# mgp25/OpenLTE

Measured on AMD Instinct MI355X. Metric: DL subframes/sec @20MHz 100RB 64QAM, full chain FFT->CE->demap->rate-unmatch->turbo(REF)->CRC (SURVEY 8d W4), higher is better.
Workload: dtype i8 IQ in, f32 FFT/CE/equaliser, i8 soft bits, i16 path metrics (differences exact modulo 2^16); 1 GPU; W4 full DL chain: 20 MHz/100 RB/64QAM, 9 allocations per subframe (8x12 PRB TBS 3240 + 1x4 PRB TBS 1064), 65536 subframes per GPU, int8 IQ in HBM; subframes_per_gpu=65536, N_ant=1, CFI=2, channel_estimate_form=compact, decoder=REF (reference-faithful, bit-exact), unique_subframes=96, streams_per_gpu=1

## Files before the change

openlte_amd/csrc/turbo.hip:

```cpp
#include <algorithm>
#include <cstring>
#include <initializer_list>
#include <type_traits>
#include <vector>

#include "plan_core.hpp"
#include "turbo_swar.h"
#include "soft_pack.h"

using namespace turbo_geom;

namespace {

constexpr uint32_t RX_NULL_AS_INT = 10000;


__device__ __forceinline__ int sbyte(uint32_t w, int k) { return (int)__builtin_amdgcn_sbfe(w, 8 * k, 8); }

typedef __attribute__((address_space(3))) const uint8_t  lds_u8_t;
typedef __attribute__((address_space(3))) const int8_t   lds_i8_t;
typedef __attribute__((address_space(3))) const uint16_t lds_u16_t;
__device__ __forceinline__ uint32_t lds_u8(uint32_t addr) { return *(lds_u8_t *)(uintptr_t)addr; }
__device__ __forceinline__ int      lds_i8(uint32_t addr) { return *(lds_i8_t *)(uintptr_t)addr; }
__device__ __forceinline__ uint32_t lds_u16(uint32_t addr) { return *(lds_u16_t *)(uintptr_t)addr; }
// ... 641 lines not shown
    __syncthreads();

    uint4 I0 = make_uint4(0, 0, 0, 0);
    if (nv > 0) {
        uint32_t idx[16];
        if constexpr (MULTI)
            load_idx16_at(reinterpret_cast<const_u32x4_t *>(reinterpret_cast<uintptr_t>(pi + 16 * (size_t)u)), nv, idx, K);
        else
            load_idx16(pi, u, nv, idx, K);
        I0 = gather16_bytes(PREP_Q0_AT, idx);
    }
    if (nv >= 0) *reinterpret_cast<uint4 *>(out.arr[3] + unit_off(tile_off, lane, u)) = I0;
    if (identity && src.hard_inputs()) {
        auto cnt4 = [](uint32_t a, uint32_t b) { return (a & 0x01010101u) + (b & 0x01010101u); };
        const uint32_t c1[4] = {cnt4(Q[1].x, Q[0].x), cnt4(Q[1].y, Q[0].y), cnt4(Q[1].z, Q[0].z), cnt4(Q[1].w, Q[0].w)};
        const uint32_t c2[4] = {cnt4(Q[2].x, I0.x), cnt4(Q[2].y, I0.y), cnt4(Q[2].z, I0.z), cnt4(Q[2].w, I0.w)};
        const uint32_t o1 = c1[0] | c1[1] | c1[2] | c1[3], o2 = c2[0] | c2[1] | c2[2] | c2[3];
        int w1max = (o1 & 0x02020202u) ? 254 : (o1 ? 127 : 0), w2max = (o2 & 0x02020202u) ? 254 : (o2 ? 127 : 0);
        block_max_i2(w1max, w2max, red_i);
        if (w1max != 0 && w2max != 0) {
            auto mag4 = [](uint32_t cnt, int W) { return W == 254 ? (cnt << 6) - ((cnt | (cnt >> 1)) & 0x01010101u) : (cnt << 7) - cnt; };
            if (nv >= 0) {
                *reinterpret_cast<uint4 *>(out.arr[4] + unit_off(tile_off, lane, u)) = make_uint4(mag4(c1[0], w1max), mag4(c1[1], w1max), mag4(c1[2], w1max), mag4(c1[3], w1max));
                *reinterpret_cast<uint4 *>(out.arr[5] + unit_off(tile_off, lane, u)) = make_uint4(mag4(c2[0], w2max), mag4(c2[1], w2max), mag4(c2[2], w2max), mag4(c2[3], w2max));
            }
            return;
        }
    }
    uint32_t w1[16], w2[16], w1m = 0, w2m = 0;
    abs_sum16(Q[1], Q[0], w1, w1m);
    abs_sum16(Q[2], I0, w2, w2m);
    int w1max = (int)w1m, w2max = (int)w2m;
    block_max_i2(w1max, w2max, red_i);
    auto closed = [](int W) { return W == 254 || W == 127; };
    auto closed16 = [](const uint32_t (&w)[16], int W) {
        uint32_t o[4];
#pragma unroll
        for (int j = 0; j < 4; j++) {
            const uint32_t p = pack4u(w[4 * j], w[4 * j + 1], w[4 * j + 2], w[4 * j + 3]);
            o[j] = W == 254 ? (p >> 1) & 0x7F7F7F7Fu : p;
        }
        return make_uint4(o[0], o[1], o[2], o[3]);
    };
    if (!(closed(w1max) && closed(w2max))) {
        const float W1 = (float)w1max, W2 = (float)w2max;
        for (uint32_t t = threadIdx.x; t < MTAB_N; t += blockDim.x) {
            const float w = (float)t;
            mtab1[t] = (int8_t)(int)(127.0f * (w / W1));
            mtab2[t] = (int8_t)(int)(127.0f * (w / W2));
        }
        __syncthreads();
    }
    if (nv >= 0) {
        *reinterpret_cast<uint4 *>(out.arr[4] + unit_off(tile_off, lane, u)) = closed(w1max) ? closed16(w1, w1max) : lookup16(0, w1);
        *reinterpret_cast<uint4 *>(out.arr[5] + unit_off(tile_off, lane, u)) = closed(w2max) ? closed16(w2, w2max) : lookup16(MTAB_N, w2);
    }
}


struct SisoPass {
    const uint8_t *in_a;
    const uint8_t *in_b;
    uint32_t      *sgn;
    uint32_t      *dec;
};
struct SisoArgs { SisoPass p[2]; };

typedef unsigned short v2u __attribute__((ext_vector_type(2)));
__device__ __forceinline__ uint32_t sign_bits(v2s n) { return __builtin_bit_cast(uint32_t, __builtin_bit_cast(v2u, n) >> 15); }

template <int S> __device__ __forceinline__ void acs_step2(v2s (&pm)[8], v2s x2, v2s y2, uint32_t &acc)
{
    const v2s mx = as_v2s(neg_mask(x2 ^ y2)), nmx = ~mx;
    const v2s uP = (x2 + y2) & nmx;
    const v2s uQ = (x2 - y2) & mx;
    const uint32_t m0p = neg_mask(x2) & 0xFFF8FFF8u;
    const v2s P2 = as_v2s(__builtin_amdgcn_bitop3_b32(as_u32(mx), m0p, 0xFFFCFFFCu, 0x06));
    const v2s Q2 = as_v2s(__builtin_amdgcn_bitop3_b32(as_u32(mx), m0p, 0xFFFCFFFCu, 0x60));
    const v2s n0 = pm[1] - pm[0], n1 = pm[3] - pm[2], n2 = pm[5] - pm[4], n3 = pm[7] - pm[6];
    constexpr uint32_t top = 0x00010001u << (15 - 4 * S);
    acc = __builtin_amdgcn_bitop3_b32(acc, neg_mask(n0), top, 0xF8);
    acc = __builtin_amdgcn_bitop3_b32(acc, neg_mask(n1), top >> 1, 0xF8);
// ... 338 lines not shown
            G = map_compose(G, map_row_shl<2>(G, MAP_ID));
            G = map_compose(G, map_row_shl<4>(G, MAP_ID));
            G = map_compose(G, map_row_shl<8>(G, MAP_ID));
            const uint32_t row = lane >> 4;
#pragma unroll
            for (int r = 1; r < 4; r++) {
                const uint2 R = make_uint2((uint32_t)__builtin_amdgcn_readlane((int)G.x, 16 * r), (uint32_t)__builtin_amdgcn_readlane((int)G.y, 16 * r));
                if (row < (uint32_t)r) G = map_compose(G, R);
            }
            const uint2    Gn  = make_uint2((uint32_t)__shfl_down((int)G.x, 1u), (uint32_t)__shfl_down((int)G.y, 1u));
            const uint32_t nxt = lane == 63 ? end : map_at(Gn, end);
            const uint32_t st  = map_at(G, end);
            const bool     pos = (nxt < st) || (nxt == st && nxt == 0);
            const uint64_t neg = __ballot(__shfl((int)(t < K && !pos), (int)turbo_swar::sign_plane_lane(lane)) != 0);
            if (lane == 0) *reinterpret_cast<uint2 *>(sgn + 2 * ch) = make_uint2((uint32_t)neg, (uint32_t)(neg >> 32));
            end = (uint32_t)__builtin_amdgcn_readlane((int)st, 0);
        }
    }
}

namespace sw = turbo_swar;
struct UnitWords { uint32_t w[5]; };
__device__ __forceinline__ UnitWords load_unit_words(const uint8_t *arr, size_t tile_off, uint32_t lane, uint32_t u)
{
    const uint4 c    = *reinterpret_cast<const uint4 *>(arr + unit_off(tile_off, lane, u));
    uint32_t    prev = 0x7F7F7F7Fu;
    if (u > 0) prev = *reinterpret_cast<const uint32_t *>(arr + unit_off(tile_off, lane, u - 1) + 12);
    return UnitWords{{prev, c.x, c.y, c.z, c.w}};
}
struct UnitSigned {
    uint32_t halo, m[4], x;
    __device__ __forceinline__ sw::SM4 word(int j) const { return sw::SM4{m[j], sw::signed_under(m[j], x, j)}; }
};
__device__ __forceinline__ UnitSigned load_unit_signed(const uint8_t *mag, const uint32_t *sgn, size_t tile_off, uint32_t lane, uint32_t nblk, uint32_t u)
{
    const UnitWords w  = load_unit_words(mag, tile_off, lane, u);
    const uint32_t *sp = sgn + (tile_off >> 5) + sw::sign_word_index(lane, nblk, u >> 1);
    const uint32_t  S = sp[0];
    uint32_t        Sb = 0;
    if ((u & 1u) == 0 && u > 0) Sb = sp[-1];
    UnitSigned r{w.w[0], {w.w[1], w.w[2], w.w[3], w.w[4]}, sw::sign_unit(S, u)};
    if (u > 0) r.halo |= sw::signed_under_flags(r.halo, sw::sign_halo(S, Sb, u));
    return r;
}
struct PermArgs { const uint8_t *M1; const uint32_t *S1;  const uint8_t *X2; uint8_t *out[2];  };

#ifndef PERM_NB
#define PERM_NB 4
#endif
static_assert(PERM_NB == PERM_BLOCKS, "a size's perm grid is a multiple of 128 workgroups (the merged decode's map granularity) only for four blocks per workgroup");
template <int NSLOT, bool MULTI = false>
__global__ __launch_bounds__(384) void k_turbo_perm(PermArgs a, uint32_t K_arg, uint32_t n_cb_arg, const uint16_t *__restrict__ pi_arg, MultiArgs ma)
{
    static_assert(NSLOT == 1, "one unit per thread");
    uint32_t K = K_arg, n_cb = n_cb_arg, bidx = blockIdx.x, grid = gridDim.x;
    size_t   seg_off = 0;
    const uint16_t *__restrict__ pi = pi_arg;
    if constexpr (MULTI) {
        const_seg_t &sg = multi_seg(ma, blockIdx.x >> 7);
        K = sg.K; n_cb = sg.n_cb; pi = (const uint16_t *)sg.pi; bidx = blockIdx.x - sg.wg_perm; grid = sg.perm_grid;
        seg_off = sg.arr_off;
    }
    extern __shared__ __attribute__((aligned(16))) int8_t smp[];
    int8_t *mtab = smp, *sm = smp + MTAB_N;
    const uint32_t Kp = kpad64(K), n_units = Kp >> 4;
    int           *red_i = reinterpret_cast<int *>(sm + Kp);
    const uint32_t u0 = threadIdx.x;
    const int      nv = (u0 < n_units) ? min(16, max(0, (int)K - 16 * (int)u0)) : -1;
    IdxRaw         praw;
    {
        const uint4 *ip = reinterpret_cast<const uint4 *>(pi + 16 * (size_t)(nv > 0 ? u0 : 0));
        const uint32_t kk = K | K << 16;
        praw.lo = ip[0];
        praw.hi = (nv > 8) ? ip[1] : make_uint4(kk, kk, kk, kk);
    }
#pragma unroll 1
    for (uint32_t it = 0; it < PERM_NB; it++) {
        const uint32_t cb = xcd_cb(bidx + it * grid, n_cb), tile = cb >> 6, lane = cb & 63;
        const size_t   tile_off = seg_off + (size_t)tile * Kp * 64;
        if (cb >= n_cb) {
            if (MULTI && cb < ((n_cb + 63u) & ~63u) && nv >= 0) {
                *reinterpret_cast<uint4 *>(a.out[0] + unit_off(tile_off, lane, u0)) = make_uint4(0, 0, 0, 0);
                *reinterpret_cast<uint4 *>(a.out[1] + unit_off(tile_off, lane, u0)) = make_uint4(0, 0, 0, 0);
            }
            continue;
        }
        uint32_t u = u0;
        asm volatile("" : "+v"(u), "+v"(praw.lo.x), "+v"(praw.lo.y), "+v"(praw.lo.z), "+v"(praw.lo.w), "+v"(praw.hi.x), "+v"(praw.hi.y), "+v"(praw.hi.z), "+v"(praw.hi.w));
        uint4          X2 = make_uint4(0, 0, 0, 0);
        if (nv >= 0) {
            const UnitSigned ua = load_unit_signed(a.M1, a.S1, tile_off, lane, n_units >> 2, u);
            uint32_t         pa = ua.halo;
            X2 = *reinterpret_cast<const uint4 *>(a.X2 + unit_off(tile_off, lane, u));
            uint32_t c1[4];
#pragma unroll
            for (int j = 0; j < 4; j++) {
                const sw::SM4  A  = ua.word(j);
                const uint32_t ja = sw::join(A);
                c1[j] = (4 * j < nv) ? sw::to_tc(sw::step3(A, sw::feedback(ja, pa))) : 0u;
                pa    = ja;
            }
            *reinterpret_cast<uint4 *>(sm + 16 * u) = make_uint4(c1[0], c1[1], c1[2], c1[3]);
        }
        __syncthreads();
        uint4 I1 = make_uint4(0, 0, 0, 0);
        if (nv > 0) {
            uint32_t idx[16];
            unpack_idx16(praw, idx);
            I1 = gather16_bytes(MTAB_N, idx);
        }
        if (nv >= 0) *reinterpret_cast<uint4 *>(a.out[0] + unit_off(tile_off, lane, u)) = I1;
        uint32_t w[16], wm = 0;
        if (nv <= 0) X2 = make_uint4(0, 0, 0, 0);
        abs_sum16(X2, I1, w, wm);
        const int   wmax = block_max_i((int)wm, red_i);
        if (wmax == 254 || wmax == 127) {
            uint32_t o[4];
#pragma unroll
            for (int j = 0; j < 4; j++) {
                const uint32_t p = pack4u(w[4 * j], w[4 * j + 1], w[4 * j + 2], w[4 * j + 3]);
                o[j] = wmax == 254 ? (p >> 1) & 0x7F7F7F7Fu : p;
            }
            if (nv >= 0) *reinterpret_cast<uint4 *>(a.out[1] + unit_off(tile_off, lane, u)) = make_uint4(o[0], o[1], o[2], o[3]);
            continue;
        }
        const float W = (float)wmax;
        for (uint32_t t = threadIdx.x; t < MTAB_N; t += blockDim.x) mtab[t] = (int8_t)(int)(127.0f * ((float)t / W));
        __syncthreads();
        if (nv >= 0) *reinterpret_cast<uint4 *>(a.out[1] + unit_off(tile_off, lane, u)) = lookup16(0, w);
        __syncthreads();
    }
}

struct VoteArgs { const uint8_t *X0, *M1, *M2, *M3; const uint32_t *S1, *S2, *S3; };

template <bool GROUP, int NSLOT, bool MULTI = false>
__global__ __launch_bounds__(384) __attribute__((amdgpu_waves_per_eu(6, 8))) void k_turbo_vote(VoteArgs a, uint32_t K_arg, uint32_t n_cb_arg, const uint16_t *__restrict__ inv_arg,
                                                    uint8_t *__restrict__ c_bits, GroupDesc g, MultiArgs ma)
{
    static_assert(NSLOT == 1, "one unit per thread");
    uint32_t K = K_arg, n_cb = n_cb_arg, bidx = blockIdx.x;
    size_t   seg_off = 0;
    const uint16_t *__restrict__ inv = inv_arg;
    if constexpr (MULTI) {
        const_seg_t &sg = multi_seg(ma, blockIdx.x >> 9);
        K = sg.K; n_cb = sg.n_cb; inv = (const uint16_t *)sg.inv2; bidx = blockIdx.x - sg.wg_cb; seg_off = sg.arr_off;
        g.desc += sg.cb_base;
    }
    extern __shared__ __attribute__((aligned(16))) int8_t sm[];
    const uint32_t cb = xcd_cb(bidx, n_cb), tile = cb >> 6, lane = cb & 63, Kp = kpad64(K), n_units = Kp >> 4;
    if (cb >= n_cb) return;
    const size_t   tile_off = seg_off + (size_t)tile * Kp * 64;
    int8_t        *d12 = sm, *bits = sm + 2 * Kp + 32;
    uint32_t      *red_u = reinterpret_cast<uint32_t *>(bits + Kp);
    const uint32_t u  = threadIdx.x;
    const int      nv = (u < n_units) ? min(16, max(0, (int)K - 16 * (int)u)) : -1;
    IdxRaw vraw;
    {
        const uint4 *ip = reinterpret_cast<const uint4 *>(inv + 16 * (size_t)(nv > 0 ? u : 0));
        vraw.lo = ip[0];
        vraw.hi = ip[1];
    }
    const uint32_t crc_w0 = (GROUP && nv > 0) ? g.crc_tab[MI_CRC_TAB_BIAS + K - 16 * u - 16] : 0u;
    v2s            s0e[4], s0o[4];
    if (threadIdx.x == 0) *reinterpret_cast<uint32_t *>(d12 + 2 * Kp) = 0u;
    if (nv >= 0) {
        const UnitSigned ua = load_unit_signed(a.M1, a.S1, tile_off, lane, n_units >> 2, u), ub = load_unit_signed(a.M2, a.S2, tile_off, lane, n_units >> 2, u),
                         uc = load_unit_signed(a.M3, a.S3, tile_off, lane, n_units >> 2, u);
        uint32_t        pa = ua.halo, pb = ub.halo, pc = uc.halo;
        const uint4    x0 = *reinterpret_cast<const uint4 *>(a.X0 + unit_off(tile_off, lane, u));
        const uint32_t x0w[4] = {x0.x, x0.y, x0.z, x0.w};
        uint32_t       dn[8];
#pragma unroll
        for (int j = 0; j < 4; j++) {
            const sw::SM4  A = ua.word(j), B = ub.word(j), B_ = uc.word(j);
            const uint32_t ja = sw::join(A), jb = sw::join(B), jc = sw::join(B_);
            const sw::SM4  F  = sw::feedback(ja, pa);
            const sw::SM4  G  = sw::feedback(jb, pb);
            const sw::SM4  G_ = sw::feedback(jc, pc);
            pa = ja; pb = jb; pc = jc;
            const uint32_t u1 = sw::step10_biased(A, B, G), n2 = sw::step11_neg_biased(B_, G_);
            const uint32_t de = sw::sub_halves(sw::even_halves(u1), sw::even_halves(n2)), dd = sw::sub_halves(sw::odd_halves(u1), sw::odd_halves(n2));
            const uint32_t x0b = x0w[j] ^ sw::HI, nc = sw::step3_neg_biased(A, F);
            s0e[j] = as_v2s(sw::sub_halves(sw::even_halves(x0b), sw::even_halves(nc)));
            s0o[j] = as_v2s(sw::sub_halves(sw::odd_halves(x0b), sw::odd_halves(nc)));
            const bool in = 4 * j < nv;
            dn[2 * j]     = in ? __builtin_amdgcn_perm(dd, de, 0x05040100u) : 0u;
            dn[2 * j + 1] = in ? __builtin_amdgcn_perm(dd, de, 0x07060302u) : 0u;
        }
        uint4 *dst = reinterpret_cast<uint4 *>(d12 + 32 * u);
        dst[0] = make_uint4(dn[0], dn[1], dn[2], dn[3]);
        dst[1] = make_uint4(dn[4], dn[5], dn[6], dn[7]);
    } else {
#pragma unroll
        for (int j = 0; j < 4; j++) s0e[j] = s0o[j] = (v2s)(0);
    }
    __syncthreads();
    uint32_t alloc = 0, tbs = 0, F = 0, crc = 0;
    if (GROUP) {
        alloc = g.desc[cb].alloc;
        tbs   = g.desc[cb].tbs;
        F     = K - tbs - 24;
    }
    if (nv > 0) {
        const uint32_t  iw[8] = {vraw.lo.x, vraw.lo.y, vraw.lo.z, vraw.lo.w, vraw.hi.x, vraw.hi.y, vraw.hi.z, vraw.hi.w};
        uint32_t        me[4], mo[4], bw[4];
#pragma unroll
        for (int j = 0; j < 4; j++) {
            const uint32_t i0 = iw[2 * j] & 0xFFFFu, i1 = iw[2 * j] >> 16, i2 = iw[2 * j + 1] & 0xFFFFu, i3 = iw[2 * j + 1] >> 16;
            const uint32_t ge = lds_u16(i0) | lds_u16(i2) << 16, go = lds_u16(i1) | lds_u16(i3) << 16;
            me[j] = as_u32((s0e[j] + as_v2s(ge)) >> 15);
            mo[j] = as_u32((s0o[j] + as_v2s(go)) >> 15);
            bw[j] = (me[j] & 0x00010001u) | (mo[j] & 0x00010001u) << 8;
        }
        if (GROUP) {
            if (!(nv == 16 && 16 * u >= F)) {
#pragma unroll
                for (int j = 0; j < 4; j++) {
                    auto ok = [&](int k) { return (k < nv && 16 * u + k >= F) ? 0xFFFFu : 0u; };
                    me[j] &= ok(4 * j) | ok(4 * j + 2) << 16;
                    mo[j] &= ok(4 * j + 1) | ok(4 * j + 3) << 16;
                }
            }
            const uint32_t GS = 0x864CFBu << 8;
            uint32_t       w = crc_w0;
#pragma unroll
            for (int k = 15; k >= 0; k--) {
                const int      j = k >> 2;
                const uint32_t m = (k & 3) == 0 ? (uint32_t)__builtin_amdgcn_sbfe(me[j], 0, 1) : (k & 3) == 1 ? (uint32_t)__builtin_amdgcn_sbfe(mo[j], 0, 1)
                                 : (k & 3) == 2 ? (uint32_t)((int)me[j] >> 31) : (uint32_t)((int)mo[j] >> 31);
                crc ^= w & m;
                if (k > 0) w = (w << 1) ^ ((uint32_t)((int)w >> 31) & GS);
            }
        }
        const uint4 pk = make_uint4(bw[0], bw[1], bw[2], bw[3]);
        if (GROUP) *reinterpret_cast<uint4 *>(bits + 16 * u) = pk;
        else {
            uint2 *o = reinterpret_cast<uint2 *>(c_bits + (size_t)cb * K + 16 * u);
            o[0] = make_uint2(pk.x, pk.y);
            if (nv > 8) o[1] = make_uint2(pk.z, pk.w);
        }
    }
    if (GROUP) {
// ... 250 lines not shown
                const uint32_t m = 0u - (((k < 4 ? lo : hi) >> (8 * (k & 3))) & 1u);
                crc ^= w & m;
                if (k > 0) w = (w << 1) ^ ((uint32_t)((int)w >> 31) & GS);
            }
            const uint32_t j = 8 * g8 - F;
            if (j < tbs) {
                if (g.packed) o[j >> 3] = (uint8_t)((((lo * 0x08040201u) >> 24) & 0xFu) << 4 | (((hi * 0x08040201u) >> 24) & 0xFu));
                else          *reinterpret_cast<uint2 *>(o + j) = make_uint2(lo, hi);
            }
        }
    } else {
        for (uint32_t j = F + threadIdx.x; j < K; j += blockDim.x) {
            const uint32_t b = c[j] & 1u;
            crc ^= b ? g.crc_tab[MI_CRC_TAB_BIAS + K - 1 - j] : 0u;
            if (j < F + tbs && !g.packed) o[j - F] = (uint8_t)b;
        }
        if (g.packed)
            for (uint32_t m = threadIdx.x; m < (tbs + 7) >> 3; m += blockDim.x) {
                uint32_t v = 0;
                for (uint32_t b = 0; b < 8; b++) v = v << 1 | ((8 * m + b < tbs) ? (c[F + 8 * m + b] & 1u) : 0u);
                o[m] = (uint8_t)v;
            }
    }
    crc = wave_xor_u(crc);
    if ((threadIdx.x & 63) == 0) red[threadIdx.x >> 6] = crc;
    __syncthreads();
    if (threadIdx.x == 0) g.status[alloc] = ((red[0] ^ red[1] ^ red[2] ^ red[3]) == 0) ? 0 : 2;
}

}


namespace {
enum { AX0, AX1, AX2, AI0, AM1, AM2, AI1, AM3 };
static_assert(sizeof(CbDesc) == CB_DESC_BYTES, "ref_scratch_bytes counts a descriptor per slot");
}

extern "C" size_t mi_lte_turbo_scratch_bytes(uint32_t K, uint32_t n_cb)
{
    const size_t n_tiles = (n_cb + 63) / 64;
    return ref_scratch_bytes(n_tiles * kpad64(K) * 64, n_tiles * 64);
}

static bool no_static_lds(std::initializer_list<const void *> kernels)
{
    hipFuncAttributes a;
    for (const void *k : kernels)
        if (hipFuncGetAttributes(&a, k) != hipSuccess || a.sharedSizeBytes != 0) return false;
    return true;
}

struct RefScratch {
    uint8_t *base;
    CbDesc  *d_desc;
    PrepOut  po;
    SisoArgs s1, s23;
    PermArgs pa;
    VoteArgs va;
    RefScratch(void *scratch, size_t arr_bytes) : base((uint8_t *)scratch)
    {
        uint8_t *arr[N_BYTE_ARRAYS];
        for (int a = 0; a < N_BYTE_ARRAYS; a++) arr[a] = base + a * arr_bytes;
        uint32_t *dec[3];
        for (int p = 0; p < 3; p++) dec[p] = (uint32_t *)(base + N_BYTE_ARRAYS * arr_bytes + p * (arr_bytes / 2));
        uint32_t *sgn[3];
        for (int p = 0; p < 3; p++) sgn[p] = (uint32_t *)(base + N_BYTE_ARRAYS * arr_bytes + 3 * (arr_bytes / 2) + p * (arr_bytes / 8));
        d_desc = (CbDesc *)(base + N_BYTE_ARRAYS * arr_bytes + 3 * (arr_bytes / 2) + 3 * (arr_bytes / 8));
        po.arr[0] = arr[AX0]; po.arr[1] = arr[AX1]; po.arr[2] = arr[AX2];
        po.arr[3] = arr[AI0]; po.arr[4] = arr[AM1]; po.arr[5] = arr[AM2];
        s1.p[0] = {arr[AX1], arr[AX0], sgn[0], dec[0]};
        s1.p[1] = s1.p[0];
        pa.M1 = arr[AM1]; pa.S1 = sgn[0]; pa.X2 = arr[AX2]; pa.out[0] = arr[AI1]; pa.out[1] = arr[AM3];
        s23.p[0] = {arr[AX2], arr[AI0], sgn[1], dec[1]};
        s23.p[1] = {arr[AX2], arr[AI1], sgn[2], dec[2]};
        va = {arr[AX0], arr[AM1], arr[AM2], arr[AM3], sgn[0], sgn[1], sgn[2]};
    }
};

template <typename Src, bool GROUP>
static int turbo_ref_run(mi_lte_ctx *ctx, Src src, uint32_t K, uint32_t n_cb, uint8_t *d_c_bits, GroupDesc gd, uint32_t e_cap = 0)
{
    TurboTables tb;
    int         rc = mi_ctx_turbo_tables(ctx, K, 0, &tb);
    if (rc != MI_LTE_OK) return rc;
    static const bool lds_ok = no_static_lds({(const void *)k_turbo_prep<Src, 1>, (const void *)k_turbo_perm<1>, (const void *)k_turbo_vote<GROUP, 1>});
    if (!lds_ok) { ctx->err = "turbo kernels were built with static LDS: absolute LDS addressing is invalid"; return MI_LTE_ERR_HIP; }
    const size_t n_tiles = (n_cb + 63) / 64, Kp = kpad64(K), arr_bytes = n_tiles * Kp * 64;
    rc = mi_ctx_reserve_scratch(ctx, ref_scratch_bytes(arr_bytes, n_tiles * 64));
    if (rc != MI_LTE_OK) return rc;
    const RefScratch sc(ctx->scratch, arr_bytes);
    const bool small = n_cb <= ctx->siso_small_max;
    if (n_cb % 64 && !small)
        MI_HIP_CHECK(ctx, hipMemsetAsync(sc.base, 0, N_BYTE_ARRAYS * arr_bytes, ctx->stream));

    if constexpr (GROUP) {
        gd.desc = src.g.desc = sc.d_desc;
        MI_LAUNCH(ctx, "k_cb_desc", k_cb_desc, dim3((n_cb + 255) / 256), dim3(256), 0, gd, n_cb, (const uint32_t *)src.nnn, sc.d_desc);
    }
    const uint32_t cb_threads = cb_width(K);
    MI_LAUNCH(ctx, "k_turbo_prep", (k_turbo_prep<Src, 1>), dim3(cb_grid(n_cb)), dim3(cb_threads), prep_lds_bytes(Kp, e_cap), src, K, n_cb, tb.d_pi, sc.po, MultiArgs{});

    auto lds_of = [&](uint32_t gpw) { return siso_small_lds_bytes(gpw, Kp); };
    if (small)
        MI_LAUNCH(ctx, "k_turbo_siso_small", k_turbo_siso_small<false>, dim3((n_cb + gpw_of(n_cb) - 1) / gpw_of(n_cb)), dim3(64), lds_of(gpw_of(n_cb)), sc.s1, K, n_cb, 0u,
                  gpw_of(n_cb), MultiArgs{});
    else
        MI_LAUNCH(ctx, "k_turbo_siso", (k_turbo_siso<false, 0>), dim3(((n_tiles + 1) / 2 + 3) / 4), dim3(256), 0, sc.s1, K, (uint32_t)n_tiles, MultiArgs{}, (const uint32_t *)nullptr);

    MI_LAUNCH(ctx, "k_turbo_perm", k_turbo_perm<1>, dim3(perm_grid_of(n_cb)), dim3(cb_threads), MTAB_N + Kp + 32, sc.pa, K, n_cb, tb.d_pi, MultiArgs{});

    if (small)
        MI_LAUNCH(ctx, "k_turbo_siso_small", k_turbo_siso_small<false>, dim3((2 * n_cb + gpw_of(2 * n_cb) - 1) / gpw_of(2 * n_cb)), dim3(64), lds_of(gpw_of(2 * n_cb)), sc.s23, K,
                  n_cb, 1u, gpw_of(2 * n_cb), MultiArgs{});
    else
        MI_LAUNCH(ctx, "k_turbo_siso", (k_turbo_siso<false, 1>), dim3((n_tiles + 3) / 4), dim3(256), 0, sc.s23, K, (uint32_t)n_tiles, MultiArgs{}, (const uint32_t *)nullptr);

    MI_LAUNCH(ctx, "k_turbo_vote", (k_turbo_vote<GROUP, 1>), dim3(cb_grid(n_cb)), dim3(cb_threads), 3 * Kp + 64, sc.va, K, n_cb, tb.d_inv2, d_c_bits, gd, MultiArgs{});
    MI_HIP_CHECK(ctx, hipGetLastError());
    ctx->last_kernels = "k_turbo_prep:1,k_turbo_siso:2,k_turbo_perm:1,k_turbo_vote:1";
    return MI_LTE_OK;
}

template <typename T>
static int turbo_ref_batch(mi_lte_ctx *ctx, const T *d_soft, uint32_t K, uint32_t n_cb, uint8_t *d_c_bits)
{
    SrcDirect<T> src{0, d_soft, nullptr};
    GroupDesc    none{};
    return turbo_ref_run<SrcDirect<T>, false>(ctx, src, K, n_cb, d_c_bits, none);
}

static int rm_rank_tables(mi_lte_ctx *ctx, uint32_t K, RmTables *out)
{
    auto it = ctx->rm_tables.find(K);
    if (it == ctx->rm_tables.end()) {
        RmTables t;
        MI_HIP_CHECK(ctx, hipMalloc((void **)&t.d_tabs, sizeof(uint16_t) * 12 * 3 * K));
        MI_HIP_CHECK(ctx, hipMalloc((void **)&t.d_nnn, sizeof(uint32_t) * 12));
        ctx->owned.push_back(t.d_tabs);
        ctx->owned.push_back(t.d_nnn);
        MI_LAUNCH(ctx, "k_rm_rank_table", k_rm_rank_table, dim3((3 * K + 255) / 256, 12), dim3(256), 0, K, t.d_tabs, t.d_nnn);
        MI_HIP_CHECK(ctx, hipGetLastError());
        it = ctx->rm_tables.emplace(K, t).first;
    }
    *out = it->second;
    return MI_LTE_OK;
}

static GroupDesc group_desc(const mi_lte_ctx *ctx, const MiDecodeIO &io, uint32_t cb_base = 0)
{
    return {io.d_allocs, io.d_cb_alloc + cb_base, io.d_e, io.d_e_off, io.d_e_len, io.d_out_bits, io.out_stride, io.d_status, ctx->d_crc_tab, io.ul ? 1u : 0u, io.packed ? 1u : 0u, io.soft_packed ? 1u : 0u};
// ... 72 lines not shown

    GroupDesc gd = group_desc(ctx, io);
    gd.desc = sc.d_desc;
    MI_LAUNCH(ctx, "k_cb_desc", k_cb_desc_multi, dim3((G.n_slots + 255) / 256), dim3(256), 0, gd, G.n_slots, d_segs, n_groups, sc.d_desc);
    SrcRateUnmatchPk src;
    src.g = gd; src.tabs = nullptr; src.nnn = nullptr; src.e_cap = 0;
    for (int c = 0; c < NCLS; c++)
        if (G.grid_cb[c]) {
            if (G.one_size[c] >= 0) {
                const MiKGroup &gr = groups[G.one_size[c]];
                TurboTables tb;
                RmTables    rt;
                if ((rc = mi_ctx_turbo_tables(ctx, gr.K, 0, &tb)) != MI_LTE_OK || (rc = rm_rank_tables(ctx, gr.K, &rt)) != MI_LTE_OK) return rc;
                SrcRateUnmatchPk s1 = src;
                s1.tabs = rt.d_tabs; s1.nnn = rt.d_nnn; s1.g.desc = sc.d_desc + gr.cb_base; s1.e_cap = G.e_cap_one[c];
                PrepOut p1 = sc.po;
                for (int a = 0; a < 6; a++) p1.arr[a] += G.off_one[c];
                MI_LAUNCH(ctx, "k_turbo_prep", (k_turbo_prep<SrcRateUnmatchPk, 1, false>), dim3(G.grid_cb[c]), dim3(64 * (c + 1)), G.lds_prep[c], s1, gr.K, gr.n_cb, (const uint16_t *)tb.d_pi,
                          p1, MultiArgs{});
                continue;
            }
            MI_LAUNCH(ctx, "k_turbo_prep", (k_turbo_prep<SrcRateUnmatchPk, 1, true>), dim3(G.grid_cb[c]), dim3(64 * (c + 1)), G.lds_prep[c], src, 0u, 0u, (const uint16_t *)nullptr, sc.po,
                      (MultiArgs{d_segs, d_map + G.map_cb[c]}));
        }
    const bool small = G.n_slots <= ctx->siso_small_max;
    auto lds_small = [&](uint32_t gpw) { return siso_small_lds_bytes(gpw, G.kp_all); };
    if (small)
        MI_LAUNCH(ctx, "k_turbo_siso_small", k_turbo_siso_small<true>, dim3(G.n_ws1), dim3(64), lds_small(G.gpw1), sc.s1, 0u, 0u, 0u, G.gpw1, (MultiArgs{d_segs, d_map + G.map_ws1}));
    else
    MI_LAUNCH(ctx, "k_turbo_siso", (k_turbo_siso<true, 0>), dim3(G.n_ord1 ? G.n_ord1 / 4 : (G.n_wv1 + 3) / 4), dim3(256), G.siso_pad1, sc.s1, 0u, G.n_wv1, (MultiArgs{d_segs, d_map + G.map_wv1}),
              G.n_ord1 ? d_map + G.ord_wv1 : (const uint32_t *)nullptr);
    for (int c = 0; c < NCLS; c++)
        if (G.grid_perm[c])
            MI_LAUNCH(ctx, "k_turbo_perm", (k_turbo_perm<1, true>), dim3(G.grid_perm[c]), dim3(64 * (c + 1)), MTAB_N + G.kp_max[c] + 32, sc.pa, 0u, 0u, (const uint16_t *)nullptr,
                      (MultiArgs{d_segs, d_map + G.map_perm[c]}));
    if (small)
        MI_LAUNCH(ctx, "k_turbo_siso_small", k_turbo_siso_small<true>, dim3(G.n_ws23), dim3(64), lds_small(G.gpw23), sc.s23, 0u, 0u, 1u, G.gpw23, (MultiArgs{d_segs, d_map + G.map_ws23}));
    else
    MI_LAUNCH(ctx, "k_turbo_siso", (k_turbo_siso<true, 1>), dim3(G.n_ord23 ? G.n_ord23 / 4 : (G.n_wv23 + 3) / 4), dim3(256), G.siso_pad23, sc.s23, 0u, G.n_wv23, (MultiArgs{d_segs, d_map + G.map_wv23}),
              G.n_ord23 ? d_map + G.ord_wv23 : (const uint32_t *)nullptr);
    for (int c = 0; c < NCLS; c++)
        if (G.grid_cb[c])
            MI_LAUNCH(ctx, "k_turbo_vote", (k_turbo_vote<true, 1, true>), dim3(G.grid_cb[c]), dim3(64 * (c + 1)), 3 * G.kp_max[c] + 64, sc.va, 0u, 0u, (const uint16_t *)nullptr,
                      (uint8_t *)nullptr, gd, (MultiArgs{d_segs, d_map + G.map_cb[c]}));
    MI_HIP_CHECK(ctx, hipGetLastError());
    return MI_LTE_OK;
}

int mi_turbo_ref_dispatch(mi_lte_ctx *ctx, const MiKGroup *groups, uint32_t n_groups, const MiDecodeIO &io, MiMultiCache *cache)
{
    std::vector<MiKGroup> take;
    if (ctx->merged_decode)
        for (uint32_t i = 0; i < n_groups; i++)
            if (mi_turbo_ref_multi_takes(groups[i].K, groups[i].e_max)) take.push_back(groups[i]);
    const bool merged = take.size() >= 2;
    int        rc;
    if (merged && (rc = mi_turbo_ref_multi(ctx, take.data(), (uint32_t)take.size(), io, cache)) != MI_LTE_OK) return rc;
    for (uint32_t i = 0; i < n_groups; i++) {
        const MiKGroup &gr = groups[i];
        if (merged && mi_turbo_ref_multi_takes(gr.K, gr.e_max)) continue;
        rc = mi_turbo_ref_group(ctx, gr, io);
        if (rc != MI_LTE_OK) return rc;
    }
    ctx->last_kernels = !merged                 ? "k_turbo_prep,k_turbo_siso,k_turbo_perm,k_turbo_vote per block size"
                        : take.size() == n_groups ? "k_cb_desc:1,k_turbo_prep,k_turbo_siso:2,k_turbo_perm,k_turbo_vote per workgroup width over all block sizes"
                                                  : "k_cb_desc:1,k_turbo_prep,k_turbo_siso:2,k_turbo_perm,k_turbo_vote per workgroup width over all block sizes but the per-size ones";
    return MI_LTE_OK;
}

void mi_multi_cache_free(MiMultiCache *cache)
{
    if (cache && cache->d_tab) (void)hipFree(cache->d_tab);
    if (cache) { cache->d_tab = nullptr; cache->cap = 0; cache->built_for.clear(); }
}

int mi_turbo_bcjr_group(mi_lte_ctx *ctx, const MiKGroup &gr, const MiDecodeIO &io, int8_t *d_soft, uint8_t *d_c_bits, uint32_t mode, uint32_t n_iter, int qpp_spec)
// ... 77 lines not shown
```

openlte_amd/csrc/turbo_plan.hpp:

```cpp
#pragma once

#include <cstddef>
#include <cstdint>
#include <vector>

#ifdef __HIPCC__
#define MI_HD __host__ __device__
#else
#define MI_HD
#endif
#ifdef __clang__
#define MI_GLOBAL_AS __attribute__((address_space(1)))
#else
#define MI_GLOBAL_AS
#endif

namespace turbo_geom {

MI_HD inline uint32_t kpad64(uint32_t K) { return (K + 63u) & ~63u; }

MI_HD inline uint32_t xcd_chunk(uint32_t n_cb) { return ((((n_cb + 63u) >> 6) + 7u) >> 3) << 6; }
MI_HD inline uint32_t xcd_cb(uint32_t b, uint32_t n_cb) { return (b & 7u) * xcd_chunk(n_cb) + (b >> 3); }
inline uint32_t cb_grid(uint32_t n_cb) { return 8 * xcd_chunk(n_cb); }

constexpr int NCLS = 6;
inline uint32_t cb_width(uint32_t K) { return ((kpad64(K) >> 4) + 63u) & ~63u; }
inline int      cb_class(uint32_t K) { return (int)(cb_width(K) >> 6) - 1; }

constexpr uint32_t PERM_BLOCKS = 4;
inline uint32_t perm_grid_of(uint32_t n_cb) { return ((cb_grid(n_cb) + PERM_BLOCKS - 1) / PERM_BLOCKS + 7u) & ~7u; }

constexpr uint32_t SMALL_G = 8;
inline uint32_t gpw_of(uint32_t n_tr) { return n_tr <= 2048 ? 1u : n_tr <= 4096 ? 2u : n_tr <= 8192 ? 4u : SMALL_G; }
inline size_t   siso_small_lds_bytes(uint32_t gpw, size_t Kp) { return sizeof(uint32_t) * gpw * (64 * 4 * 2 + (Kp >> 5) * 4); }

constexpr uint32_t QTAB_N = 4096;
constexpr uint32_t QTAB_HALF = 2048;
constexpr uint32_t MTAB_N = 256;
constexpr uint32_t PREP_RED_AT = 2 * MTAB_N, PREP_E_AT = PREP_RED_AT + 64, PREP_QTAB_AT = PREP_E_AT, PREP_Q0_AT = PREP_QTAB_AT + QTAB_N;
MI_HD constexpr uint32_t prep_lds_bytes(uint32_t Kp, uint32_t e_cap) { return PREP_E_AT + (e_cap > QTAB_N + Kp ? e_cap : QTAB_N + Kp); }
inline uint32_t stage_cap(uint32_t e_max_bytes) { return (e_max_bytes + 16u + 63u) & ~63u; }
inline bool prep_stages(uint32_t K, uint32_t cap) { return prep_lds_bytes(kpad64(K), cap) <= 48 * 1024; }
inline uint32_t merged_e_cap(uint32_t K, uint32_t e_max_bytes)
{
    const uint32_t cap = stage_cap(e_max_bytes), cap_w = (uint32_t)((15 * (size_t)(K + 4) / 4 + 64 + 63) & ~(size_t)63);
    return prep_stages(K, cap) ? (kpad64(K) <= 1024 ? (cap < cap_w ? cap : cap_w) : cap) : cap_w;
}

inline bool mi_turbo_ref_multi_takes(uint32_t K, uint32_t e_max_bytes) { return (e_max_bytes + (3 * K - 81) - 1) / (3 * K - 81) <= 258; }
inline bool mi_turbo_ref_reads_packed(uint32_t K, uint32_t e_max_bytes) { return mi_turbo_ref_multi_takes(K, e_max_bytes) || prep_stages(K, stage_cap(e_max_bytes)); }

constexpr int    N_BYTE_ARRAYS = 8;
constexpr size_t CB_DESC_BYTES = 32;
inline size_t ref_scratch_bytes(size_t arr_bytes, size_t n_slots) { return N_BYTE_ARRAYS * arr_bytes + 3 * (arr_bytes / 2) + 3 * (arr_bytes / 8) + ((n_slots + 63) & ~(size_t)63) * CB_DESC_BYTES; }

}

struct MiKGroup { uint32_t K, n_cb, cb_base, e_max; };

struct KSeg {
    uint32_t        K, n_cb, cb_base, n_tiles;
    uint32_t        wg_cb;
    uint32_t        wg_perm, perm_grid;
    uint32_t        e_cap;
    uint32_t        wv1, wv23;
    uint64_t        arr_off;
    MI_GLOBAL_AS const uint16_t *pi, *inv2, *tabs;
    MI_GLOBAL_AS const uint32_t *nnn;
    uint32_t        ws1, ws23;
    uint64_t        pad;
};
static_assert(sizeof(KSeg) == 96, "KSeg is read with scalar loads: keep it a multiple of 16 bytes");
struct MultiArgs { const KSeg *segs; const uint32_t *map; };

struct MiMultiGeom {
    uint64_t arr_bytes = 0;
    uint32_t n_slots = 0, n_wv1 = 0, n_wv23 = 0;
    uint32_t grid_cb[6] = {0}, grid_perm[6] = {0}, lds_prep[6] = {0}, kp_max[6] = {0};
    uint32_t map_cb[6] = {0}, map_perm[6] = {0}, map_wv1 = 0, map_wv23 = 0;
    uint32_t ord_wv1 = 0, ord_wv23 = 0, n_ord1 = 0, n_ord23 = 0;
    uint32_t siso_pad1 = 0, siso_pad23 = 0;
    int      one_size[6] = {-1, -1, -1, -1, -1, -1};
    uint64_t off_one[6] = {0}; uint32_t e_cap_one[6] = {0};
    uint32_t map_ws1 = 0, map_ws23 = 0, n_ws1 = 0, n_ws23 = 0, gpw1 = 1, gpw23 = 1, kp_all = 0;
    size_t   map_off = 0;
// ... 5 lines not shown
```

openlte_amd/csrc/turbo_swar.h:

```cpp
#pragma once

#include <cstddef>
#include <cstdint>

#ifdef __HIPCC__
#define SWAR_FN __host__ __device__ __forceinline__
#else
#define SWAR_FN inline
#endif

namespace turbo_swar {

constexpr uint32_t HI = 0x80808080u, LO7 = 0x7F7F7F7Fu, ONES = 0x01010101u, EVEN = 0x00FF00FFu;

SWAR_FN uint32_t alignbit(uint32_t hi, uint32_t lo, uint32_t sh)
{
#if defined(__HIP_DEVICE_COMPILE__)
    return __builtin_amdgcn_alignbit(hi, lo, sh);
#else
    return (uint32_t)((((uint64_t)hi << 32) | lo) >> sh);
#endif
}
SWAR_FN uint32_t sub_halves(uint32_t a, uint32_t b)
{
// ... 63 lines not shown
    const uint32_t m = half_sum(a.m, b.m);
    return SM4{m, (a.s ^ b.s) & (m + LO7) & HI};
}

SWAR_FN uint32_t delay2(uint32_t cur, uint32_t prev) { return alignbit(cur, prev, 16); }
SWAR_FN uint32_t delay3(uint32_t cur, uint32_t prev) { return alignbit(cur, prev, 8); }
SWAR_FN SM4 feedback(uint32_t cur_joined, uint32_t prev_joined)
{
    const uint32_t d2 = delay2(cur_joined, prev_joined), d3 = delay3(cur_joined, prev_joined);
    const uint32_t x = d2 ^ d3;
    const uint32_t m = (d2 & d3 & LO7) + ((x >> 1) & 0x3F3F3F3Fu);
    return SM4{m, x & (m + LO7) & HI};
}

SWAR_FN SM4 step3(const SM4 &A, const SM4 &F) { return soft_xor(A, F); }
SWAR_FN uint32_t step3_neg_biased(const SM4 &A, const SM4 &F) { return biased(half_sum(A.m, F.m), A.s ^ F.s ^ HI); }

SWAR_FN uint32_t avg_biased(uint32_t xb, uint32_t yb) { return (xb & yb) + (((xb ^ yb) >> 1) & LO7); }

SWAR_FN uint32_t step10_biased(const SM4 &A, const SM4 &B, const SM4 &G)
{
    const uint32_t mx = B.s ^ G.s, tm = mx >> 7, m7 = mx - tm;
    const uint32_t y  = (A.m & m7) | (B.m & ~m7);
    const uint32_t w  = avg_biased(G.m | HI, biased(y, mx & (A.s ^ B.s)));
    return (w ^ (m7 | mx)) + tm;
}
SWAR_FN uint32_t step11_neg_biased(const SM4 &B, const SM4 &G)
{
    const uint32_t mx = B.s ^ G.s, tm = mx >> 7, m7 = mx - tm;
    const uint32_t w  = avg_biased(B.m | HI, biased(G.m, mx & B.s));
    return (w ^ ~(m7 | mx)) + (tm ^ ONES);
}

SWAR_FN uint32_t traceback_entry(uint32_t byte, uint32_t cur)
{
    uint32_t sgn = 0;
    for (int k = 0; k < 2; k++) {
        const uint32_t nib = k ? byte >> 4 : byte & 15u;
        const uint32_t j = cur & 3u, bit = (nib >> (3 - j)) & 1u, st = 2 * j + bit;
        const bool     pos = (cur < st) || (cur == st && cur == 0);
        if (!pos) sgn |= k ? 1u << 16 : 1u << 24;
        cur = st;
    }
    return cur | sgn;
}

}
```

Measured before the change: 3.048 million subframes/s.

## Compute M3 magnitude normalisation inside vote kernel instead of perm kernel

Moves the |X2|+|I1| sum, block max and magnitude-table normalisation from the perm kernel into the vote kernel. The AM3 scratch array and its global write/read round trip go away, and the perm kernel loses a block reduction and a barrier. The vote kernel now loads X2 and I1 and builds halos via DPP lane shifts and memory reads at wave boundaries. It gains an extra block reduction, possible table-building syncs, and more register pressure.

```diff
diff --git a/openlte_amd/csrc/turbo.hip b/openlte_amd/csrc/turbo.hip
--- a/openlte_amd/csrc/turbo.hip
+++ b/openlte_amd/csrc/turbo.hip
@@ -697,22 +697,18 @@
     abs_sum16(Q[2], I0, w2, w2m);
     int w1max = (int)w1m, w2max = (int)w2m;
     block_max_i2(w1max, w2max, red_i);
-    auto closed = [](int W) { return W == 254 || W == 127; };
+    auto closed = [](int W) { return turbo_swar::mag_closed(W); };
     auto closed16 = [](const uint32_t (&w)[16], int W) {
         uint32_t o[4];
 #pragma unroll
-        for (int j = 0; j < 4; j++) {
-            const uint32_t p = pack4u(w[4 * j], w[4 * j + 1], w[4 * j + 2], w[4 * j + 3]);
-            o[j] = W == 254 ? (p >> 1) & 0x7F7F7F7Fu : p;
-        }
+        for (int j = 0; j < 4; j++) o[j] = turbo_swar::mag_closed_word(pack4u(w[4 * j], w[4 * j + 1], w[4 * j + 2], w[4 * j + 3]), W);
         return make_uint4(o[0], o[1], o[2], o[3]);
     };
     if (!(closed(w1max) && closed(w2max))) {
         const float W1 = (float)w1max, W2 = (float)w2max;
         for (uint32_t t = threadIdx.x; t < MTAB_N; t += blockDim.x) {
-            const float w = (float)t;
-            mtab1[t] = (int8_t)(int)(127.0f * (w / W1));
-            mtab2[t] = (int8_t)(int)(127.0f * (w / W2));
+            mtab1[t] = (int8_t)turbo_swar::mag_entry(t, W1);
+            mtab2[t] = (int8_t)turbo_swar::mag_entry(t, W2);
         }
         __syncthreads();
     }
@@ -1117,18 +1113,25 @@
     uint32_t halo, m[4], x;
     __device__ __forceinline__ sw::SM4 word(int j) const { return sw::SM4{m[j], sw::signed_under(m[j], x, j)}; }
 };
+struct UnitSigns { uint32_t S, Sb; };
+__device__ __forceinline__ UnitSigns load_unit_signs(const uint32_t *sgn, size_t tile_off, uint32_t lane, uint32_t nblk, uint32_t u)
+{
+    const uint32_t *sp = sgn + (tile_off >> 5) + sw::sign_word_index(lane, nblk, u >> 1);
+    UnitSigns       r{sp[0], 0u};
+    if ((u & 1u) == 0 && u > 0) r.Sb = sp[-1];
+    return r;
+}
+__device__ __forceinline__ UnitSigned unit_signed(const UnitWords &w, const UnitSigns &s, uint32_t u)
+{
+    UnitSigned r{w.w[0], {w.w[1], w.w[2], w.w[3], w.w[4]}, sw::sign_unit(s.S, u)};
+    if (u > 0) r.halo |= sw::signed_under_flags(r.halo, sw::sign_halo(s.S, s.Sb, u));
+    return r;
+}
 __device__ __forceinline__ UnitSigned load_unit_signed(const uint8_t *mag, const uint32_t *sgn, size_t tile_off, uint32_t lane, uint32_t nblk, uint32_t u)
 {
-    const UnitWords w  = load_unit_words(mag, tile_off, lane, u);
-    const uint32_t *sp = sgn + (tile_off >> 5) + sw::sign_word_index(lane, nblk, u >> 1);
-    const uint32_t  S = sp[0];
-    uint32_t        Sb = 0;
-    if ((u & 1u) == 0 && u > 0) Sb = sp[-1];
-    UnitSigned r{w.w[0], {w.w[1], w.w[2], w.w[3], w.w[4]}, sw::sign_unit(S, u)};
-    if (u > 0) r.halo |= sw::signed_under_flags(r.halo, sw::sign_halo(S, Sb, u));
-    return r;
-}
-struct PermArgs { const uint8_t *M1; const uint32_t *S1;  const uint8_t *X2; uint8_t *out[2];  };
+    return unit_signed(load_unit_words(mag, tile_off, lane, u), load_unit_signs(sgn, tile_off, lane, nblk, u), u);
+}
+struct PermArgs { const uint8_t *M1; const uint32_t *S1;  uint8_t *I1; };
 
 #ifndef PERM_NB
 #define PERM_NB 4
@@ -1146,10 +1149,8 @@
         K = sg.K; n_cb = sg.n_cb; pi = (const uint16_t *)sg.pi; bidx = blockIdx.x - sg.wg_perm; grid = sg.perm_grid;
         seg_off = sg.arr_off;
     }
-    extern __shared__ __attribute__((aligned(16))) int8_t smp[];
-    int8_t *mtab = smp, *sm = smp + MTAB_N;
+    extern __shared__ __attribute__((aligned(16))) int8_t sm[];
     const uint32_t Kp = kpad64(K), n_units = Kp >> 4;
-    int           *red_i = reinterpret_cast<int *>(sm + Kp);
     const uint32_t u0 = threadIdx.x;
     const int      nv = (u0 < n_units) ? min(16, max(0, (int)K - 16 * (int)u0)) : -1;
     IdxRaw         praw;
@@ -1164,19 +1165,15 @@
         const uint32_t cb = xcd_cb(bidx + it * grid, n_cb), tile = cb >> 6, lane = cb & 63;
         const size_t   tile_off = seg_off + (size_t)tile * Kp * 64;
         if (cb >= n_cb) {
-            if (MULTI && cb < ((n_cb + 63u) & ~63u) && nv >= 0) {
-                *reinterpret_cast<uint4 *>(a.out[0] + unit_off(tile_off, lane, u0)) = make_uint4(0, 0, 0, 0);
-                *reinterpret_cast<uint4 *>(a.out[1] + unit_off(tile_off, lane, u0)) = make_uint4(0, 0, 0, 0);
-            }
+            if (MULTI && cb < ((n_cb + 63u) & ~63u) && nv >= 0)
+                *reinterpret_cast<uint4 *>(a.I1 + unit_off(tile_off, lane, u0)) = make_uint4(0, 0, 0, 0);
             continue;
         }
         uint32_t u = u0;
         asm volatile("" : "+v"(u), "+v"(praw.lo.x), "+v"(praw.lo.y), "+v"(praw.lo.z), "+v"(praw.lo.w), "+v"(praw.hi.x), "+v"(praw.hi.y), "+v"(praw.hi.z), "+v"(praw.hi.w));
-        uint4          X2 = make_uint4(0, 0, 0, 0);
         if (nv >= 0) {
             const UnitSigned ua = load_unit_signed(a.M1, a.S1, tile_off, lane, n_units >> 2, u);
             uint32_t         pa = ua.halo;
-            X2 = *reinterpret_cast<const uint4 *>(a.X2 + unit_off(tile_off, lane, u));
             uint32_t c1[4];
 #pragma unroll
             for (int j = 0; j < 4; j++) {
@@ -1192,32 +1189,14 @@
         if (nv > 0) {
             uint32_t idx[16];
             unpack_idx16(praw, idx);
-            I1 = gather16_bytes(MTAB_N, idx);
-        }
-        if (nv >= 0) *reinterpret_cast<uint4 *>(a.out[0] + unit_off(tile_off, lane, u)) = I1;
-        uint32_t w[16], wm = 0;
-        if (nv <= 0) X2 = make_uint4(0, 0, 0, 0);
-        abs_sum16(X2, I1, w, wm);
-        const int   wmax = block_max_i((int)wm, red_i);
-        if (wmax == 254 || wmax == 127) {
-            uint32_t o[4];
-#pragma unroll
-            for (int j = 0; j < 4; j++) {
-                const uint32_t p = pack4u(w[4 * j], w[4 * j + 1], w[4 * j + 2], w[4 * j + 3]);
-                o[j] = wmax == 254 ? (p >> 1) & 0x7F7F7F7Fu : p;
-            }
-            if (nv >= 0) *reinterpret_cast<uint4 *>(a.out[1] + unit_off(tile_off, lane, u)) = make_uint4(o[0], o[1], o[2], o[3]);
-            continue;
-        }
-        const float W = (float)wmax;
-        for (uint32_t t = threadIdx.x; t < MTAB_N; t += blockDim.x) mtab[t] = (int8_t)(int)(127.0f * ((float)t / W));
+            I1 = gather16_bytes(0, idx);
+        }
+        if (nv >= 0) *reinterpret_cast<uint4 *>(a.I1 + unit_off(tile_off, lane, u)) = I1;
         __syncthreads();
-        if (nv >= 0) *reinterpret_cast<uint4 *>(a.out[1] + unit_off(tile_off, lane, u)) = lookup16(0, w);
-        __syncthreads();
-    }
-}
-
-struct VoteArgs { const uint8_t *X0, *M1, *M2, *M3; const uint32_t *S1, *S2, *S3; };
+    }
+}
+
+struct VoteArgs { const uint8_t *X0, *M1, *M2, *X2, *I1; const uint32_t *S1, *S2, *S3; };
 
 template <bool GROUP, int NSLOT, bool MULTI = false>
 __global__ __launch_bounds__(384) __attribute__((amdgpu_waves_per_eu(6, 8))) void k_turbo_vote(VoteArgs a, uint32_t K_arg, uint32_t n_cb_arg, const uint16_t *__restrict__ inv_arg,
@@ -1236,7 +1215,7 @@
     const uint32_t cb = xcd_cb(bidx, n_cb), tile = cb >> 6, lane = cb & 63, Kp = kpad64(K), n_units = Kp >> 4;
     if (cb >= n_cb) return;
     const size_t   tile_off = seg_off + (size_t)tile * Kp * 64;
-    int8_t        *d12 = sm, *bits = sm + 2 * Kp + 32;
+    int8_t        *mtab = sm, *d12 = sm + MTAB_N, *bits = d12 + 2 * Kp + 32;
     uint32_t      *red_u = reinterpret_cast<uint32_t *>(bits + Kp);
     const uint32_t u  = threadIdx.x;
     const int      nv = (u < n_units) ? min(16, max(0, (int)K - 16 * (int)u)) : -1;
@@ -1249,11 +1228,52 @@
     const uint32_t crc_w0 = (GROUP && nv > 0) ? g.crc_tab[MI_CRC_TAB_BIAS + K - 16 * u - 16] : 0u;
     v2s            s0e[4], s0o[4];
     if (threadIdx.x == 0) *reinterpret_cast<uint32_t *>(d12 + 2 * Kp) = 0u;
+    uint32_t  p3[5] = {0u, 0u, 0u, 0u, 0u}, w3max = 0, h1 = 0x7F7F7F7Fu, h2 = 0x7F7F7F7Fu;
+    UnitSigns s1{}, s2{}, s3{};
+    uint4     x0 = make_uint4(0, 0, 0, 0), m1 = x0, m2 = x0;
+    const bool halo_mem = (u & 63u) == 0 && u > 0;
     if (nv >= 0) {
-        const UnitSigned ua = load_unit_signed(a.M1, a.S1, tile_off, lane, n_units >> 2, u), ub = load_unit_signed(a.M2, a.S2, tile_off, lane, n_units >> 2, u),
-                         uc = load_unit_signed(a.M3, a.S3, tile_off, lane, n_units >> 2, u);
+        uint4 X2 = *reinterpret_cast<const uint4 *>(a.X2 + unit_off(tile_off, lane, u)), I1 = *reinterpret_cast<const uint4 *>(a.I1 + unit_off(tile_off, lane, u));
+        m1 = *reinterpret_cast<const uint4 *>(a.M1 + unit_off(tile_off, lane, u));
+        m2 = *reinterpret_cast<const uint4 *>(a.M2 + unit_off(tile_off, lane, u));
+        s1 = load_unit_signs(a.S1, tile_off, lane, n_units >> 2, u);
+        s2 = load_unit_signs(a.S2, tile_off, lane, n_units >> 2, u);
+        s3 = load_unit_signs(a.S3, tile_off, lane, n_units >> 2, u);
+        x0 = *reinterpret_cast<const uint4 *>(a.X0 + unit_off(tile_off, lane, u));
+        if (halo_mem) {
+            const size_t   ho = unit_off(tile_off, lane, u - 1) + 12;
+            const uint32_t hxb = bias4(*reinterpret_cast<const uint32_t *>(a.X2 + ho)), hib = bias4(*reinterpret_cast<const uint32_t *>(a.I1 + ho));
+            h1 = *reinterpret_cast<const uint32_t *>(a.M1 + ho);
+            h2 = *reinterpret_cast<const uint32_t *>(a.M2 + ho);
+            p3[0] = pack4u(abs_sum2<0>(hxb, hib), abs_sum2<1>(hxb, hib), abs_sum2<2>(hxb, hib), abs_sum2<3>(hxb, hib));
+        }
+        if (nv == 0) X2 = I1 = make_uint4(0, 0, 0, 0);
+        uint32_t w[16];
+        abs_sum16(X2, I1, w, w3max);
+#pragma unroll
+        for (int j = 0; j < 4; j++) p3[1 + j] = pack4u(w[4 * j], w[4 * j + 1], w[4 * j + 2], w[4 * j + 3]);
+    }
+    w3max = (uint32_t)wave_max_i((int)w3max);
+    if ((threadIdx.x & 63) == 0) red_u[threadIdx.x >> 6] = w3max;
+    __syncthreads();
+    int W3 = (int)red_u[0];
+    for (uint32_t w = 1; w < (blockDim.x >> 6); w++) W3 = max(W3, (int)red_u[w]);
+    if (!sw::mag_closed(W3)) {
+        for (uint32_t t = threadIdx.x; t < MTAB_N; t += blockDim.x) mtab[t] = (int8_t)sw::mag_entry(t, (float)W3);
+        __syncthreads();
+    }
+    if (nv >= 0) {
+        auto tab = [](uint32_t w) { return lds_u8(w); };
+        uint32_t m3[4], h3 = 0x7F7F7F7Fu;
+#pragma unroll
+        for (int j = 0; j < 4; j++) m3[j] = sw::mag_word(p3[1 + j], W3, tab);
+        if (halo_mem) h3 = sw::mag_word(p3[0], W3, tab);
+        auto left = [](uint32_t v) { return (uint32_t)__builtin_amdgcn_update_dpp(0, (int)v, 0x138, 0xF, 0xF, false); };
+        const uint32_t l1 = left(m1.w), l2 = left(m2.w), l3 = left(m3[3]);
+        if (u & 63u) { h1 = l1; h2 = l2; h3 = l3; }
+        const UnitSigned ua = unit_signed(UnitWords{{h1, m1.x, m1.y, m1.z, m1.w}}, s1, u), ub = unit_signed(UnitWords{{h2, m2.x, m2.y, m2.z, m2.w}}, s2, u),
+                         uc = unit_signed(UnitWords{{h3, m3[0], m3[1], m3[2], m3[3]}}, s3, u);
         uint32_t        pa = ua.halo, pb = ub.halo, pc = uc.halo;
-        const uint4    x0 = *reinterpret_cast<const uint4 *>(a.X0 + unit_off(tile_off, lane, u));
         const uint32_t x0w[4] = {x0.x, x0.y, x0.z, x0.w};
         uint32_t       dn[8];
 #pragma unroll
@@ -1293,7 +1313,7 @@
 #pragma unroll
         for (int j = 0; j < 4; j++) {
             const uint32_t i0 = iw[2 * j] & 0xFFFFu, i1 = iw[2 * j] >> 16, i2 = iw[2 * j + 1] & 0xFFFFu, i3 = iw[2 * j + 1] >> 16;
-            const uint32_t ge = lds_u16(i0) | lds_u16(i2) << 16, go = lds_u16(i1) | lds_u16(i3) << 16;
+            const uint32_t ge = lds_u16(MTAB_N + i0) | lds_u16(MTAB_N + i2) << 16, go = lds_u16(MTAB_N + i1) | lds_u16(MTAB_N + i3) << 16;
             me[j] = as_u32((s0e[j] + as_v2s(ge)) >> 15);
             mo[j] = as_u32((s0o[j] + as_v2s(go)) >> 15);
             bw[j] = (me[j] & 0x00010001u) | (mo[j] & 0x00010001u) << 8;
@@ -1610,7 +1630,7 @@
 
 
 namespace {
-enum { AX0, AX1, AX2, AI0, AM1, AM2, AI1, AM3 };
+enum { AX0, AX1, AX2, AI0, AM1, AM2, AI1 };
 static_assert(sizeof(CbDesc) == CB_DESC_BYTES, "ref_scratch_bytes counts a descriptor per slot");
 }
 
@@ -1648,10 +1668,10 @@
         po.arr[3] = arr[AI0]; po.arr[4] = arr[AM1]; po.arr[5] = arr[AM2];
         s1.p[0] = {arr[AX1], arr[AX0], sgn[0], dec[0]};
         s1.p[1] = s1.p[0];
-        pa.M1 = arr[AM1]; pa.S1 = sgn[0]; pa.X2 = arr[AX2]; pa.out[0] = arr[AI1]; pa.out[1] = arr[AM3];
+        pa.M1 = arr[AM1]; pa.S1 = sgn[0]; pa.I1 = arr[AI1];
         s23.p[0] = {arr[AX2], arr[AI0], sgn[1], dec[1]};
         s23.p[1] = {arr[AX2], arr[AI1], sgn[2], dec[2]};
-        va = {arr[AX0], arr[AM1], arr[AM2], arr[AM3], sgn[0], sgn[1], sgn[2]};
+        va = {arr[AX0], arr[AM1], arr[AM2], arr[AX2], pa.I1, sgn[0], sgn[1], sgn[2]};
     }
 };
 
@@ -1685,7 +1705,7 @@
     else
         MI_LAUNCH(ctx, "k_turbo_siso", (k_turbo_siso<false, 0>), dim3(((n_tiles + 1) / 2 + 3) / 4), dim3(256), 0, sc.s1, K, (uint32_t)n_tiles, MultiArgs{}, (const uint32_t *)nullptr);
 
-    MI_LAUNCH(ctx, "k_turbo_perm", k_turbo_perm<1>, dim3(perm_grid_of(n_cb)), dim3(cb_threads), MTAB_N + Kp + 32, sc.pa, K, n_cb, tb.d_pi, MultiArgs{});
+    MI_LAUNCH(ctx, "k_turbo_perm", k_turbo_perm<1>, dim3(perm_grid_of(n_cb)), dim3(cb_threads), perm_lds_bytes(Kp), sc.pa, K, n_cb, tb.d_pi, MultiArgs{});
 
     if (small)
         MI_LAUNCH(ctx, "k_turbo_siso_small", k_turbo_siso_small<false>, dim3((2 * n_cb + gpw_of(2 * n_cb) - 1) / gpw_of(2 * n_cb)), dim3(64), lds_of(gpw_of(2 * n_cb)), sc.s23, K,
@@ -1693,7 +1713,7 @@
     else
         MI_LAUNCH(ctx, "k_turbo_siso", (k_turbo_siso<false, 1>), dim3((n_tiles + 3) / 4), dim3(256), 0, sc.s23, K, (uint32_t)n_tiles, MultiArgs{}, (const uint32_t *)nullptr);
 
-    MI_LAUNCH(ctx, "k_turbo_vote", (k_turbo_vote<GROUP, 1>), dim3(cb_grid(n_cb)), dim3(cb_threads), 3 * Kp + 64, sc.va, K, n_cb, tb.d_inv2, d_c_bits, gd, MultiArgs{});
+    MI_LAUNCH(ctx, "k_turbo_vote", (k_turbo_vote<GROUP, 1>), dim3(cb_grid(n_cb)), dim3(cb_threads), vote_lds_bytes(Kp), sc.va, K, n_cb, tb.d_inv2, d_c_bits, gd, MultiArgs{});
     MI_HIP_CHECK(ctx, hipGetLastError());
     ctx->last_kernels = "k_turbo_prep:1,k_turbo_siso:2,k_turbo_perm:1,k_turbo_vote:1";
     return MI_LTE_OK;
@@ -1832,7 +1852,7 @@
               G.n_ord1 ? d_map + G.ord_wv1 : (const uint32_t *)nullptr);
     for (int c = 0; c < NCLS; c++)
         if (G.grid_perm[c])
-            MI_LAUNCH(ctx, "k_turbo_perm", (k_turbo_perm<1, true>), dim3(G.grid_perm[c]), dim3(64 * (c + 1)), MTAB_N + G.kp_max[c] + 32, sc.pa, 0u, 0u, (const uint16_t *)nullptr,
+            MI_LAUNCH(ctx, "k_turbo_perm", (k_turbo_perm<1, true>), dim3(G.grid_perm[c]), dim3(64 * (c + 1)), perm_lds_bytes(G.kp_max[c]), sc.pa, 0u, 0u, (const uint16_t *)nullptr,
                       (MultiArgs{d_segs, d_map + G.map_perm[c]}));
     if (small)
         MI_LAUNCH(ctx, "k_turbo_siso_small", k_turbo_siso_small<true>, dim3(G.n_ws23), dim3(64), lds_small(G.gpw23), sc.s23, 0u, 0u, 1u, G.gpw23, (MultiArgs{d_segs, d_map + G.map_ws23}));
@@ -1841,7 +1861,7 @@
               G.n_ord23 ? d_map + G.ord_wv23 : (const uint32_t *)nullptr);
     for (int c = 0; c < NCLS; c++)
         if (G.grid_cb[c])
-            MI_LAUNCH(ctx, "k_turbo_vote", (k_turbo_vote<true, 1, true>), dim3(G.grid_cb[c]), dim3(64 * (c + 1)), 3 * G.kp_max[c] + 64, sc.va, 0u, 0u, (const uint16_t *)nullptr,
+            MI_LAUNCH(ctx, "k_turbo_vote", (k_turbo_vote<true, 1, true>), dim3(G.grid_cb[c]), dim3(64 * (c + 1)), vote_lds_bytes(G.kp_max[c]), sc.va, 0u, 0u, (const uint16_t *)nullptr,
                       (uint8_t *)nullptr, gd, (MultiArgs{d_segs, d_map + G.map_cb[c]}));
     MI_HIP_CHECK(ctx, hipGetLastError());
     return MI_LTE_OK;
diff --git a/openlte_amd/csrc/turbo_plan.hpp b/openlte_amd/csrc/turbo_plan.hpp
--- a/openlte_amd/csrc/turbo_plan.hpp
+++ b/openlte_amd/csrc/turbo_plan.hpp
@@ -39,6 +39,8 @@
 constexpr uint32_t MTAB_N = 256;
 constexpr uint32_t PREP_RED_AT = 2 * MTAB_N, PREP_E_AT = PREP_RED_AT + 64, PREP_QTAB_AT = PREP_E_AT, PREP_Q0_AT = PREP_QTAB_AT + QTAB_N;
 MI_HD constexpr uint32_t prep_lds_bytes(uint32_t Kp, uint32_t e_cap) { return PREP_E_AT + (e_cap > QTAB_N + Kp ? e_cap : QTAB_N + Kp); }
+MI_HD constexpr uint32_t perm_lds_bytes(uint32_t Kp) { return Kp; }
+MI_HD constexpr uint32_t vote_lds_bytes(uint32_t Kp) { return MTAB_N + 3 * Kp + 64; }
 inline uint32_t stage_cap(uint32_t e_max_bytes) { return (e_max_bytes + 16u + 63u) & ~63u; }
 inline bool prep_stages(uint32_t K, uint32_t cap) { return prep_lds_bytes(kpad64(K), cap) <= 48 * 1024; }
 inline uint32_t merged_e_cap(uint32_t K, uint32_t e_max_bytes)
@@ -50,7 +52,7 @@
 inline bool mi_turbo_ref_multi_takes(uint32_t K, uint32_t e_max_bytes) { return (e_max_bytes + (3 * K - 81) - 1) / (3 * K - 81) <= 258; }
 inline bool mi_turbo_ref_reads_packed(uint32_t K, uint32_t e_max_bytes) { return mi_turbo_ref_multi_takes(K, e_max_bytes) || prep_stages(K, stage_cap(e_max_bytes)); }
 
-constexpr int    N_BYTE_ARRAYS = 8;
+constexpr int    N_BYTE_ARRAYS = 7;
 constexpr size_t CB_DESC_BYTES = 32;
 inline size_t ref_scratch_bytes(size_t arr_bytes, size_t n_slots) { return N_BYTE_ARRAYS * arr_bytes + 3 * (arr_bytes / 2) + 3 * (arr_bytes / 8) + ((n_slots + 63) & ~(size_t)63) * CB_DESC_BYTES; }
 
diff --git a/openlte_amd/csrc/turbo_swar.h b/openlte_amd/csrc/turbo_swar.h
--- a/openlte_amd/csrc/turbo_swar.h
+++ b/openlte_amd/csrc/turbo_swar.h
@@ -119,6 +119,15 @@
     return (w ^ ~(m7 | mx)) + (tm ^ ONES);
 }
 
+SWAR_FN uint8_t  mag_entry(uint32_t w, float W) { return (uint8_t)(int8_t)(int)(127.0f * ((float)w / W)); }
+SWAR_FN bool     mag_closed(int W) { return W == 254 || W == 127; }
+SWAR_FN uint32_t mag_closed_word(uint32_t p, int W) { return W == 254 ? (p >> 1) & LO7 : p; }
+template <typename Tab> SWAR_FN uint32_t mag_word(uint32_t p, int W, Tab tab)
+{
+    if (mag_closed(W)) return mag_closed_word(p, W);
+    return (uint32_t)tab(p & 0xFFu) | (uint32_t)tab((p >> 8) & 0xFFu) << 8 | (uint32_t)tab((p >> 16) & 0xFFu) << 16 | (uint32_t)tab(p >> 24) << 24;
+}
+
 SWAR_FN uint32_t traceback_entry(uint32_t byte, uint32_t cur)
 {
     uint32_t sgn = 0;
```

Result: slower. 3.003 million subframes/s (-1.5%).
